# rvolden/C3POa

Measured on AMD Instinct MI355X. Metric: R2C2 reads->consensus/sec, higher is better.
Workload: dtype int32

## Files before the change

c3poa_amd/csrc/c3_api.hip:

```cpp
#include "c3_dev.h"
#include "c3_args.h"
#include <algorithm>
#include <cstddef>
#include <cstdio>
#include <cstring>
#include <string>
#include <vector>

extern "C" void c3k_launch_conk(const ConkArgs*, int, int, int, hipStream_t);
extern "C" void c3k_launch_adapter(const AdapterArgs*, int, hipStream_t);
extern "C" void c3k_launch_pairwise(const uint8_t*, int, const uint8_t*, int, const uint8_t*, int, uint8_t*, uint8_t*, int*, hipStream_t);
extern "C" void c3k_launch_match_index(const char*, const int*, int, int, const char*, const long long*, int*, hipStream_t);
extern "C" void c3k_launch_demux(const uint8_t*, int, const uint8_t*, int, int, int, int32_t*, uint8_t*, hipStream_t);
extern "C" void c3k_launch_peaks(const PeaksArgs*, int, hipStream_t);
extern "C" int c3k_peaks_blocks_per_cu(void);
extern "C" void c3k_launch_poa(const PoaArgs*, int, int, int, hipStream_t);
extern "C" void c3k_launch_prep(const PrepArgs*, int, hipStream_t);
extern "C" void c3k_launch_window(const WinArgs*, int, hipStream_t);
extern "C" void c3k_launch_stitch(const StitchArgs*, int, hipStream_t);
extern "C" void c3k_launch_zero(const ZeroArgs*, int, hipStream_t);
extern "C" void c3k_launch_zero_long(const ZeroArgs*, int, hipStream_t);
extern "C" void c3k_launch_zero_finish(const ZeroArgs*, int, hipStream_t);
extern "C" void c3k_launch_qv(const QvArgs*, int, hipStream_t);
extern "C" int c3k_qv_lds_max(void);
// ... 506 lines not shown
  if ((rc = run_zero(h))) return rc;
  const int n = h->n;
  h->work.clear();
  for (int i = 0; i < n; ++i) if (h->sum[i].status == C3_ST_OK && h->sum[i].n_sub >= 1) h->work.push_back(i);
  if (n < (1 << 24)) {
    const size_t m = h->work.size();
    std::vector<uint64_t> keys(m), tmp(m);
    for (size_t k = 0; k < m; ++k) {
      const int i = h->work[k];
      const uint64_t cost = (uint64_t)h->sum[i].sum_sub * (uint64_t)h->sum[i].n_sub;
      keys[k] = ((((uint64_t)1 << 40) - 1 - cost) << 24) | (uint64_t)i;
    }
    uint64_t* src = keys.data(); uint64_t* dst = tmp.data();
    for (int pass = 0; pass < 4; ++pass) {
      const int sh = 24 + 10 * pass;
      size_t cnt[1025] = {0};
      for (size_t k = 0; k < m; ++k) ++cnt[((src[k] >> sh) & 1023) + 1];
      for (int b = 0; b < 1024; ++b) cnt[b + 1] += cnt[b];
      for (size_t k = 0; k < m; ++k) dst[cnt[(src[k] >> sh) & 1023]++] = src[k];
      std::swap(src, dst);
    }
    for (size_t k = 0; k < m; ++k) h->work[k] = (int)(src[k] & 0xffffff);
  } else {
    std::stable_sort(h->work.begin(), h->work.end(), [&](int x, int y) {
      long cx = (long)h->sum[x].sum_sub * h->sum[x].n_sub, cy = (long)h->sum[y].sum_sub * h->sum[y].n_sub; return cx > cy; });
  }
  HIPCHK(h->d_work.ensure(sizeof(int) * std::max<size_t>(h->work.size(), 1)));
  if (!h->work.empty()) HIPCHK(hipMemcpyAsync(h->d_work.p, h->work.data(), sizeof(int) * h->work.size(), hipMemcpyHostToDevice, h->stream));
  return 0;
}

static int launch_poa(c3_handle* h, const int* d_work, int nw, int Ncap, int K, int Pcap, long long cells, int* d_overflow, int* d_overflow16, int waves_per_cu, int wide_ring) {
  const size_t N = (size_t)Ncap;
  const int NI = 19;
  cells = (cells + 15) & ~15LL;
  cells = (cells + 63) & ~63LL;
  const bool w32 = d_overflow16 == nullptr || getenv("C3_DEBUG_POA32");
  const long long far = w32 ? cells : cells >> 2;
  const size_t per_slot = N * (NI * 4 + 8 + 5 + 32 + 4 * C3_JUMP_LEVELS) + N * K * 12 + (size_t)cells * 2 + (size_t)far * 16 + (size_t)Pcap * 4;
  const int slots = auto_slots(h, h->cfg.slots_poa, per_slot, nw, waves_per_cu);
  HIPCHK(h->s_poa_i.ensure(sizeof(int) * N * NI * slots)); HIPCHK(h->s_poa_nk.ensure(sizeof(int) * N * K * 3 * slots));
  HIPCHK(h->s_poa_cells.ensure(((size_t)cells * 2 + (size_t)far * 16) * slots + 256)); HIPCHK(h->s_poa_b.ensure(N * 5 * slots)); HIPCHK(h->s_poa_sc.ensure(sizeof(long long) * N * slots));
  HIPCHK(h->s_poa_desc.ensure(sizeof(uint4) * 2 * N * slots));
  HIPCHK(h->s_poa_jump.ensure(sizeof(int) * C3_JUMP_LEVELS * N * slots));
  HIPCHK(h->s_poa_path.ensure(sizeof(int) * (size_t)Pcap * slots));
  PoaArgs a; memset(&a, 0, sizeof(a));
  a.b = dev_batch(h); a.info = h->d_info.as<C3Info>(); a.p = dev_params(h->cfg);
  a.counter = h->d_counter.as<int>(); a.work = d_work; a.n_work = nw;
  a.ibase = h->s_poa_i.as<int>(); a.ebase = h->s_poa_nk.as<int>(); a.cellsb = h->s_poa_cells.as<char>();
  a.bbase = h->s_poa_b.as<uint8_t>(); a.score = h->s_poa_sc.as<long long>();
  a.Ncap = Ncap; a.K = K; a.Pcap = Pcap; a.cells_cap = (int)cells; a.desc = h->s_poa_desc.as<uint4>(); a.jump = h->s_poa_jump.as<int>();
  a.pbase = h->s_poa_path.as<int>(); a.overflow = d_overflow; a.overflow16 = d_overflow16;
  if (const char* e = getenv("C3_DEBUG_POA_RBSPAN")) a.rb_span = std::max(3300, atoi(e));
  a.draft = h->d_draft.as<uint8_t>(); a.tpos = h->d_tpos.as<int32_t>();
  a.msa_dbg = nullptr; a.msa_off = nullptr; a.msa_len = nullptr;
  if (h->debug_msa) { a.msa_dbg = h->d_msa.as<uint8_t>(); a.msa_off = h->d_msa_off.as<int64_t>(); a.msa_len = h->d_msa_len.as<int>(); }
  a.phases = (unsigned long long*)(h->d_counter.as<char>() + 64);
  DBG("poa: nw=%d Ncap=%d K=%d cells=%lld slots=%d (%.1f MB per slot)%s\n", nw, Ncap, K, cells, slots, per_slot / 1048576.0, d_overflow ? "" : (d_overflow16 ? " [full-size pass]" : " [32-bit pass]"));
  c3k_launch_poa(&a, slots, w32 ? 1 : 0, wide_ring, h->stream);
  HIPCHK(hipGetLastError());
  return 0;
}

static int run_poa(c3_handle* h) {
  const int nw = (int)h->work.size();
  HIPCHK(h->d_draft.ensure((size_t)h->total + 64)); HIPCHK(h->d_tpos.ensure(sizeof(int32_t) * (size_t)h->total + 64));
  HIPCHK(h->d_cons.ensure((size_t)h->total + 64));
  HIPCHK(hipMemsetAsync(h->d_tpos.p, 0xff, sizeof(int32_t) * (size_t)h->total, h->stream));
  if (nw == 0) return 0;
  int max_sum = 0, max_ns = 0, max_q = 0;
  for (int i : h->work) { max_sum = std::max(max_sum, h->sum[i].sum_sub); max_ns = std::max(max_ns, h->sum[i].n_sub); max_q = std::max(max_q, h->sum[i].max_sub); }
  const int Ncap_full = max_sum + 8, K = max_ns + 1, Pcap = max_sum + 8;
  const int w = h->cfg.poa_band_b + (int)(h->cfg.poa_band_f * max_q);
  long long cells_full = (long long)(2 * max_q + 2) * (2 * w + 1 + max_q / 5);
  if (max_ns < 2) cells_full = 64;
  if (cells_full > 0x7fffff00LL) cells_full = 0x7fffff00LL;
  const double nodes_typ = (double)max_q * (1.0 + 0.15 * std::max(0, max_ns - 1));
  int Ncap = (int)std::min<double>(Ncap_full, 1.3 * nodes_typ + 256);
  long long cells = std::min<long long>(cells_full, (long long)(1.5 * nodes_typ * (2 * w + 12)) + 4096);
  if (const char* e_ = getenv("C3_DEBUG_POA_SMALL")) { Ncap = std::min(Ncap_full, std::max(64, atoi(e_))); cells = std::min<long long>(cells_full, 16LL * Ncap); }
  if (h->debug_msa) {
    std::vector<int64_t> mo(h->n + 1, 0);
    for (int i = 0; i < h->n; ++i) mo[i + 1] = mo[i] + (int64_t)h->sum[i].n_sub * (h->sum[i].sum_sub + 2);
    HIPCHK(h->d_msa.ensure((size_t)mo[h->n] + 64)); HIPCHK(h->d_msa_off.ensure(sizeof(int64_t) * (h->n + 1))); HIPCHK(h->d_msa_len.ensure(sizeof(int) * h->n));
    HIPCHK(hipMemcpyAsync(h->d_msa_off.p, mo.data(), sizeof(int64_t) * (h->n + 1), hipMemcpyHostToDevice, h->stream));
    HIPCHK(hipMemsetAsync(h->d_msa_len.p, 0, sizeof(int) * h->n, h->stream));
    HIPCHK(hipStreamSynchronize(h->stream));
  }
  HIPCHK(h->d_overflow.ensure(sizeof(int) * 2 * (size_t)nw));
  HIPCHK(hipMemsetAsync(h->d_counter.p, 0, 4, h->stream));
  HIPCHK(hipMemsetAsync(h->d_counter.as<char>() + 16, 0, 240, h->stream));
  int wide_ring = (max_q > 1792 || 2 * w + 1 + 24 > 128) ? 1 : 0;
  if (const char* e_ = getenv("C3_DEBUG_POA_WIDE")) wide_ring = atoi(e_) ? 1 : 0;
  int* ovA = h->d_overflow.as<int>(); int* ovB = h->d_overflow.as<int>() + nw;
  int rc = launch_poa(h, h->d_work.as<int>(), nw, Ncap, K, Pcap, cells, ovA, ovB, 24, wide_ring);
  if (rc) return rc;
  h->n_poa_redo = 0; h->n_poa_redo16 = 0;
  {
    int cnt[8];
    HIPCHK(hipMemcpyAsync(cnt, h->d_counter.p, 32, hipMemcpyDeviceToHost, h->stream));
    HIPCHK(hipStreamSynchronize(h->stream));
    if (cnt[4] > 0) {
      h->n_poa_redo = cnt[4];
      HIPCHK(hipMemsetAsync(h->d_counter.p, 0, 4, h->stream));
      if ((rc = launch_poa(h, ovA, cnt[4], Ncap_full, K, Pcap, cells_full, nullptr, ovB, 24, wide_ring))) return rc;
      HIPCHK(hipMemcpyAsync(cnt, h->d_counter.p, 32, hipMemcpyDeviceToHost, h->stream));
// ... 751 lines not shown
```

c3poa_amd/csrc/c3_args.h:

```cpp
#pragma once
#include "c3_dev.h"

struct ConkArgs {
  C3Batch b; const uint8_t* sp_codes; const int* sp_len; int32_t* track; C3Info* info; int* counter;
  int match, mismatch, penalty;
  int n_spl; int32_t* scan;
};
struct PeaksArgs {
  C3Batch b; const int32_t* track; C3Info* info; double* bufA; double* bufB; int32_t* cand; uint8_t* cstate;
  int32_t* raw_peaks; int32_t* n_raw; const int* sp_len; double coef[64]; int64_t maxL; int window, iters, min_dist;
  int* queue;
};
struct PoaArgs {
  C3Batch b; C3Info* info; C3Params p; int* counter; const int* work; int n_work;
  int* ibase; int* ebase; char* cellsb; uint8_t* bbase; long long* score;
  int Ncap, K, Pcap, cells_cap;
  uint8_t* draft; int32_t* tpos; uint8_t* msa_dbg; const int64_t* msa_off; int* msa_len;
  unsigned long long* phases; uint4* desc; int* jump;
  int* pbase;
  int* overflow;
  int* overflow16;
  int rb_span;
};
struct WLayer { int qbeg, len, begin, end; };
struct WinRec { int rid, w, n_layers, blen, tgs, out_len, polished, pad_; };
struct PrepArgs {
  C3Batch b; C3Info* info; C3Params p; int* counter; const int* work; int n_work;
  const uint8_t* draft; int32_t* tpos; int32_t* eH; uint8_t* eD; int64_t ecap; int* lw_first; int* lw_last; int NLcap, NWcap;
  WinRec* wrec; WLayer* wlay; int* win_base; int* n_windows; int wcap;
};
struct WinArgs {
  C3Batch b; C3Params p; int* counter; int n_win; const WinRec* wrec_in; WinRec* wrec; const WLayer* wlay; int NLcap;
  const uint8_t* draft;
  uint8_t* base; int* ibase; int* ebase; long long* score;
  int32_t* H; uint16_t* D; uint4* rdesc; int Ncap, K; long long hcap; uint8_t* wout; int wout_cap;
  int Lcap;
  unsigned long long* phases;
  int band_mode;
  const int* wlist; const int* n_win_dev; int* ovf_list;
};
#define W_CNT_OVF 48
#define W_CNT_Q2 49
struct StitchArgs {
  C3Batch b; C3Info* info; const int* work; int n_work; const WinRec* wrec; const int* win_base; const uint8_t* wout; int wout_cap; char* cons;
  const uint8_t* zflag;
};
struct AdapterArgs {
  C3Batch b; C3Params p; int* counter;
  const uint8_t* ad_codes; const int* ad_len; int n_ad;
  uint8_t* D; long long dcap;
  int32_t* out;
};

struct ZeroArgs {
  C3Batch b; C3Info* info; C3Params p; int* counter; const int* work; int n_work;
  uint8_t* D; long long dcap;
  int4* zinfo; uint8_t* zflag;
  const uint8_t* draft; char* cons;
  uint8_t* S; long long scap; int zk;
};

struct ZlLayout { long long ck, dir, car, total; };
__host__ __device__ inline ZlLayout c3_zl_layout(long long n0, long long n1, long long K) {
  ZlLayout l;
  l.ck = 0;
  l.dir = (n1 + K - 1) / K * (n0 + 1) * 8;
  l.car = (l.dir + (n1 < K ? n1 : K) * (n0 + 1) + 15) & ~15LL;
  l.total = (l.car + n1 * 12 + 255) & ~255LL;
  return l;
}
struct QvArgs {
  int n_reads; const C3Info* info; const uint32_t* pk; const int64_t* woff; const uint8_t* qual; const int64_t* off;
  const char* cons; char* qv;
  int sa_np, sa_n; const int64_t* sa_woff; const int64_t* sa_off; const int32_t* sa_mode;
  uint32_t* dirs; long long dir_words;
// ... 5 lines not shown
```

c3poa_amd/csrc/k_poa.hip:

```cpp
#include "c3_dev.h"
#include "c3_args.h"
#include <type_traits>

#define WSYNC() __syncthreads()
#define EI(v, k) ((size_t)(k) * (size_t)c.Ncap + (size_t)(v))
#define C3_POA_NI 19
#define SRC 0
#define SNK 1


struct Ctx {
  int* I; int* E; char* C; uint8_t* B8; long long* score_; uint4* desc_; int* jump_; int* path_;
  int K, n, Ncap, cells_cap;
  int far_shift;
  int osel;
  int rb_span;
  const uint32_t* pk;
#ifdef C3_DEBUG_PUNT
  unsigned long long* dbg;
#endif
#define CTX_I(name, k) __device__ __forceinline__ int* name() const { return I + (size_t)(k) * Ncap; }
  CTX_I(n_in, 0) CTX_I(n_out, 1) CTX_I(grp, 2) CTX_I(index, 5) CTX_I(gfirst, 6) CTX_I(glast, 7)
  CTX_I(rem, 8) CTX_I(mpl, 9) CTX_I(mpr, 10) CTX_I(rowm, 11)  CTX_I(anchor, 14) CTX_I(col, 15)
  CTX_I(col2t, 16) CTX_I(nxt, 17) CTX_I(foff, 18)
#undef CTX_I
  __device__ __forceinline__ int* order() const { return I + (size_t)(3 + osel) * Ncap; }
  __device__ __forceinline__ int* order2() const { return I + (size_t)(4 - osel) * Ncap; }
  __device__ __forceinline__ int* in_from() const { return E; }
  __device__ __forceinline__ int* out_to() const { return E + (size_t)Ncap * K; }
  __device__ __forceinline__ int* out_w() const { return E + 2 * (size_t)Ncap * K; }
  __device__ __forceinline__ int far_cap() const { return cells_cap >> far_shift; }
  __device__ __forceinline__ int32_t* H() const { return (int32_t*)(C + 2 * (size_t)cells_cap); }
  __device__ __forceinline__ int32_t* E1() const { return (int32_t*)(C + 2 * (size_t)cells_cap + 4 * (size_t)far_cap()); }
  __device__ __forceinline__ int32_t* E2() const { return (int32_t*)(C + 2 * (size_t)cells_cap + 8 * (size_t)far_cap()); }
  __device__ __forceinline__ uint32_t* D() const { return (uint32_t*)(C + 2 * (size_t)cells_cap + 12 * (size_t)far_cap()); }
  __device__ __forceinline__ uint8_t* D8() const { return (uint8_t*)C; }
  __device__ __forceinline__ uint8_t* P8() const { return (uint8_t*)(C + (size_t)cells_cap); }
  __device__ __forceinline__ uint8_t* base() const { return B8; }
  __device__ __forceinline__ uint8_t* rows2() const { return B8 + (size_t)Ncap; }
  __device__ __forceinline__ long long* score() const { return score_; }
  __device__ __forceinline__ uint4* descA() const { return desc_; }
  __device__ __forceinline__ uint4* descB() const { return desc_ + (size_t)Ncap; }
  __device__ __forceinline__ int* jump() const { return jump_; }
  __device__ __forceinline__ int* path() const { return path_; }
};

__device__ __forceinline__ void g_add_edge(Ctx& c, int u, int v, int w) {
  const int K = c.K;
  for (int k = 0; k < c.n_out()[u]; ++k)
    if (c.out_to()[EI(u, k)] == v) { c.out_w()[EI(u, k)] += w; return; }
  int no = c.n_out()[u], ni = c.n_in()[v];
  c.out_to()[EI(u, no)] = v; c.out_w()[EI(u, no)] = w; c.n_out()[u] = no + 1;
  c.in_from()[EI(v, ni)] = u; c.n_in()[v] = ni + 1;
}

#ifndef GU
#define GU 2
#endif
__device__ void g_blocks(Ctx& c, int lane) {
  int gprev = -1;
  for (int i0 = 0; i0 < c.n; i0 += 64 * GU) {
    int v[GU], r[GU];
#pragma unroll
    for (int u = 0; u < GU; ++u) { const int i = i0 + 64 * u + lane; v[u] = i < c.n ? c.order()[i] : -1; }
#pragma unroll
    for (int u = 0; u < GU; ++u) r[u] = v[u] >= 0 ? c.grp()[v[u]] : -2;
#pragma unroll
    for (int u = 0; u < GU; ++u) {
      const int i = i0 + 64 * u + lane;
// ... 153 lines not shown
  const int w = wave_first(P.band_b + (int)(P.band_f * (double)Q));
  const int le1_8 = e1_8 * lane, le2_8 = e2_8 * lane;
#define le1 (le1_8 << 6)
#define le2 (le2_8 << 6)
  const int lo1_8 = le1_8 + o1_8, lo2_8 = le2_8 + o2_8;
  const bool qlds = WIDE || Q <= PQW_N * 16;
  poa_sweep_desc(c, lane, Q, qlds, PR);
  int qwb = 0;
  auto stage_query = [&](int from) {
    for (int i = lane; i < PQW && from + 16 * i < Q; i += 64) {
      const long long b0 = (long long)qb + from + 16 * i;
      const unsigned w0 = c.pk[b0 >> 4], w1 = c.pk[(b0 >> 4) + 1];
      Lqpk[i] = __builtin_amdgcn_alignbit(w1, w0, (unsigned)(b0 & 15) * 2);
    }
  };
  if (qlds) stage_query(0);
  if (!W32) { unsigned* r32 = (unsigned*)&L.ring[0]; for (int i = lane; i < 3 * RING_CELLS / 2; i += 64) r32[i] = NEG16 | (NEG16 << 16); }
  WSYNC();
  PH_MARK(0)
  int u_beg = 0, u_end = -1, u_left = 0, u_right = 0, u_ncell = 0;
  int u_b8 = 0;
  int u_nfar = 0;
  int pH = NEG16, pE1 = NEG16, pE2 = NEG16;
  bool pv_ok = false;
  int gacc = 0xffff;
  int punt = 0;
  const int lane4 = lane * 4;
  unsigned short* const LH = &L.ring[0]; unsigned short* const LE1 = &L.ring[RING_CELLS]; unsigned short* const LE2 = &L.ring[2 * RING_CELLS];
#ifdef C3_EXP_SBAND
#define UNI(x)
#else
#define UNI(x) asm volatile("" : "+v"(x))
#endif
#ifdef C3_PHASE_PROF
  unsigned long long row_t0 = __builtin_readcyclecounter();
#endif
  int slot = PR - 1;
  for (int ib = 0; ib < n; ib += 64) {
  uint4 dA = c.descA()[min(ib + lane, n - 1)], dB = c.descB()[min(ib + lane, n - 1)];
  asm volatile("" : "+v"(dA.x), "+v"(dA.y), "+v"(dA.z), "+v"(dA.w), "+v"(dB.x), "+v"(dB.y), "+v"(dB.z), "+v"(dB.w));
  const int cnt = min(64, n - ib);
  for (int li = 0; li < cnt; ++li) {
    const int idx = ib + li;
    slot = slot == PR - 1 ? 0 : slot + 1;
    const int fl = __builtin_amdgcn_readlane(dA.z, li);
    if ((fl >> 19) & 1) { pv_ok = false; continue; }
    const int qr = __builtin_amdgcn_readlane(dA.w, li);
    const int vb = fl & 0xff;
    const bool far = W32 || ((fl >> 16) & 1);
    if (WIDE && qr + w + 72 > qwb + PQW * 16 && qwb + PQW * 16 < Q) {
      qwb = max(0, qr - w - 320) & ~15;
      WSYNC(); stage_query(qwb); WSYNC();
    }
    if (!W32 && ((fl >> 18) & 1) && pv_ok) {
      UNI(u_beg); UNI(u_end); UNI(u_left); UNI(u_right); UNI(u_ncell);
      const bool nonempty = u_end >= u_beg;
      const int mplv = nonempty ? u_left + 1 : INT32_MAX / 2, mprv = nonempty ? u_right + 1 : 0;
      const int beg = max(max(0, min(mplv, qr) - w), u_beg);
      int end = min(min(Q, max(mprv, qr) + w), u_end + 1);
      end = max(end, beg - 1);
      const int wd = end - beg + 1, sh = beg - u_beg;
      if (__builtin_amdgcn_ballot_w64(((int)((unsigned)(wd - 1) < 64u) & (int)(wd + sh <= 64) & ((int)(sh >= 1) | (int)(u_end - u_beg < 63)) & (int)(u_ncell + 64 <= c.cells_cap) & (int)(!far || u_nfar + 64 <= c.far_cap()) & (int)(!WIDE || (max(beg - 1, 0) >= qwb && end <= qwb + PQW * 16))) != 0) != 0) {
        const int ro = u_ncell;
        const int j = beg + lane;
        const bool act = lane < wd;
        const int jq = max(j - 1, 0) - (WIDE ? qwb : 0);
        const unsigned qw_ = Lqpk[min(jq >> 4, PQW - 1)];
        const int a_p = lane4 + sh * 4, a_d = a_p - 4;
        const int hd = __builtin_amdgcn_ds_bpermute(a_d, pH), hp = __builtin_amdgcn_ds_bpermute(a_p, pH);
        const int e1p = __builtin_amdgcn_ds_bpermute(a_p, pE1), e2p = __builtin_amdgcn_ds_bpermute(a_p, pE2);
        const int qc = (int)((qw_ >> ((jq & 15) * 2)) & 3);
        const int M = hd + ((vb == qc) ? mt8 + 2 : mm8 + 2);
        const int E1t = maxu16(hp - (oe1_8 - 1), e1p - e1_8);
        const int E2t = maxu16(hp - (oe2_8 - 2), e2p - e2_8);
        const int E1c = E1t & ~7, E2c = E2t & ~7;
        const int k2 = maxu16(maxu16(M, E1c + 1), E2c);
        const int ht = k2 & ~7;
        const int htm = act ? ht : NEG2_16;
        int s1 = htm + le1_8, s2 = htm + le2_8, s3 = htm;
        wave_scan_max3(s1, s2, s3);
        const int px1 = wave_shr1(s1, NEG2_16), px2 = wave_shr1(s2, NEG2_16);
        const int htl = wave_shr1(htm, NEG16);
        const int f1 = px1 - lo1_8, f2 = px2 - lo2_8;
        const int k3 = maxu16(maxu16(ht + 2, f1 + 1), f2);
        const int h = k3 & ~7;
        unsigned d = ((unsigned)E1t & 1u) | ((unsigned)E2t & 2u) | (((unsigned)k2 & 3u) << 2) | (((unsigned)k3 & 3u) << 4);
        d |= (((unsigned)(htl - oe1_8 - f1)) >> 25) & 64u;
        d |= (((unsigned)(htl - oe2_8 - f2)) >> 24) & 128u;
        const int rb = __builtin_amdgcn_readlane(s3, 63);
        const unsigned long long mxm = __ballot(htm == rb);
        const int left = beg + __builtin_ctzll(mxm), right = beg + (63 - __builtin_clzll(mxm));
        pH = maxu16(act ? h : NEG16, FLOOR16); pE1 = act ? E1c : NEG16; pE2 = act ? E2c : NEG16;
        int nb8 = u_b8;
        if ((unsigned)(rb - RB_LO16) > (unsigned)c.rb_span) {
          const int m1 = rb - BIAS16, fl1 = FLOOR16 + max(m1, 0);
          nb8 += m1; punt |= (int)(rb < GLO16);
          pH = act ? maxu16(h, fl1) - m1 : NEG16; pE1 = act ? maxu16(E1c, fl1) - m1 : NEG16; pE2 = act ? maxu16(E2c, fl1) - m1 : NEG16;
        }
        gacc = minu16(gacc, pH - (ZHI16 + 1));
#ifdef C3_DEBUG_PUNT
        if (pH > ZHI16 && pH < GLO16) { atomicAdd(c.dbg + 8, 1ull); atomicMax(c.dbg + 9, ((unsigned long long)(65535 - pH) << 40) | ((unsigned long long)idx << 16) | ((unsigned long long)lane << 8) | (unsigned long long)(wd & 255)); atomicMax(c.dbg + 10, ((unsigned long long)(65535 - pH) << 40) | ((unsigned long long)(unsigned short)rb << 16) | (unsigned)(sh & 255) << 8 | (unsigned)(u_end - u_beg + 1)); }
#endif
        c.D8()[(unsigned)(ro + lane)] = (uint8_t)d;
        { const int cb = slot * PWT + PADL + lane;
          LH[cb] = (unsigned short)pH; LE1[cb] = (unsigned short)pE1; LE2[cb] = (unsigned short)pE2;
#pragma unroll
          for (int f = 1; f < NCHMAX; ++f) { LH[cb + 64 * f] = NEG16; LE1[cb + 64 * f] = NEG16; LE2[cb + 64 * f] = NEG16; }
        }
        if (lane == 0) {
          L.meta[slot] = make_int4(beg, end, left, right); L.base8[slot] = nb8;
          int off = 3 * idx; UNI(off);
          int* rm = c.rowm() + off; rm[0] = beg; rm[1] = end; rm[2] = ro;
        }
        if (far) {
          const int fo = wave_first(u_nfar);
          if (act) { c.H()[fo + lane] = cv_16to9(pH, nb8); c.E1()[fo + lane] = cv_16to9(pE1, nb8); c.E2()[fo + lane] = cv_16to9(pE2, nb8); }
          if (lane == 0) { c.mpl()[idx] = left; c.mpr()[idx] = right; c.foff()[idx] = fo; }
          u_nfar = fo + wave_first(wd);
        }
        u_beg = beg; u_end = end; u_left = left; u_right = right; u_ncell = ro + wd; u_b8 = nb8;
#ifdef C3_PHASE_PROF
        { unsigned long long t_ = __builtin_readcyclecounter(); ph_acc_[8] += t_ - row_t0; row_t0 = t_; }
#endif
        continue;
      }
    }
    const int v = __builtin_amdgcn_readlane(dA.x, li);
    const int nin = (fl >> 8) & 0xff;
    const bool ovf = (fl >> 17) & 1;
    const int p0 = __builtin_amdgcn_readlane(dB.x, li), p1 = __builtin_amdgcn_readlane(dB.y, li);
    const int p2 = __builtin_amdgcn_readlane(dB.z, li), p3 = __builtin_amdgcn_readlane(dB.w, li);
    const int psl = __builtin_amdgcn_readlane(dA.y, li);
    const int ps0 = psl & 15, ps1 = (psl >> 4) & 15, ps2 = (psl >> 8) & 15, ps3 = (psl >> 12) & 15;
#define PRED_IDX(k) ((k) == 0 ? p0 : (k) == 1 ? p1 : (k) == 2 ? p2 : (k) == 3 ? p3 : c.index()[c.in_from()[EI(v, (k))]])
#define PRED_SLOT(k) ((k) == 0 ? ps0 : (k) == 1 ? ps1 : (k) == 2 ? ps2 : ps3)
    int ncell = wave_first(u_ncell);
    if (!W32 && C3_NEAR && !ovf && qlds && v != SRC && idx - p0 < PR && (nin < 2 || idx - p1 < PR) && (nin < 3 || idx - p2 < PR) && (nin < 4 || idx - p3 < PR)) {
      auto near_body = [&](auto NPc, auto NCHc) -> bool {
      constexpr int NP = decltype(NPc)::value, NCH = decltype(NCHc)::value;
      UNI(u_ncell);
      const int BIGB = 1 << 28;
      int4 m_[NP]; int b8_[NP], sl_[NP];
#pragma unroll
      for (int k = 0; k < NP; ++k) { sl_[k] = k < nin ? PRED_SLOT(k) : 0; m_[k] = L.meta[sl_[k]]; b8_[k] = L.base8[sl_[k]]; }
      int pb_[NP], dk_[NP];
      int mplv = INT32_MAX / 2, mprv = 0, minb = INT32_MAX, maxe = INT32_MIN, wmax = 0, dabs = 0;
#pragma unroll
      for (int k = 0; k < NP; ++k) {
        const bool has = k < nin;
        const int b = has ? m_[k].x : BIGB, e = has ? m_[k].y : -BIGB;
        pb_[k] = b;
        dk_[k] = has ? b8_[k] - b8_[0] : 0;
        dabs = max(dabs, max(dk_[k], -dk_[k]));
        minb = min(minb, b); maxe = max(maxe, e + 1); wmax = max(wmax, e - b);
        const bool ne = e >= b;
        mplv = ne ? min(mplv, m_[k].z + 1) : mplv; mprv = ne ? max(mprv, m_[k].w + 1) : mprv;
      }
      const int beg = max(max(0, min(mplv, qr) - w), minb);
      int end = min(min(Q, max(mprv, qr) + w), maxe);
      end = max(end, beg - 1);
      const int wd = end - beg + 1;
      if (__builtin_amdgcn_ballot_w64(((int)((unsigned)(wd - 1) < (unsigned)(64 * NCH)) & (int)(wmax < PW) & (int)(dabs < 2048) & (int)(u_ncell + 64 * NCH <= c.cells_cap) & (int)(!far || u_nfar + 64 * NCH <= c.far_cap()) & (int)(!WIDE || (max(beg - 1, 0) >= qwb && end <= qwb + PQW * 16))) != 0) == 0) return false;
      const int ro = u_ncell;
      const int W8 = wave_first(b8_[0]);
      int cM[NP], c1o[NP], c1x[NP], c2o[NP], c2x[NP], sb_[NP];
#pragma unroll
      for (int k = 0; k < NP; ++k) {
        cM[k] = dk_[k] + (3 - k);
        c1o[k] = dk_[k] - oe1_8 + (7 - 2 * k); c1x[k] = dk_[k] - e1_8 + (6 - 2 * k);
        c2o[k] = dk_[k] - oe2_8 + (7 - 2 * k); c2x[k] = dk_[k] - e2_8 + (6 - 2 * k);
        sb_[k] = sl_[k] * PWT + PADL - pb_[k];
      }
      int carry1 = 0, carry2 = 0, prev_ht = NEG16;
      int best = 0, left = 0, right = 0;
      int cH[NCH], cE1[NCH], cE2[NCH];
#pragma unroll
      for (int ch = 0; ch < NCH; ++ch) {
        const int c0 = 64 * ch;
        const int j = beg + c0 + lane;
// ... 30 lines not shown
        const int htl = wave_shr1(htm, prev_ht);
        const int f1 = px1 - o1_8 - cl1, f2 = px2 - o2_8 - cl2;
        if (NCH > 1) { carry1 = max(carry1, wave_bcast(s1, 63)); carry2 = max(carry2, wave_bcast(s2, 63)); prev_ht = wave_bcast(htm, 63); }
        const int k3 = maxu16(maxu16(ht + 2, f1 + 1), f2);
        const int h = k3 & ~7;
        d |= (((unsigned)k3 & 3u) << 4);
        d |= (((unsigned)(htl - oe1_8 - f1)) >> 25) & 64u;
        d |= (((unsigned)(htl - oe2_8 - f2)) >> 24) & 128u;
        c.D8()[(unsigned)(ro + c0 + lane)] = (uint8_t)d; c.P8()[(unsigned)(ro + c0 + lane)] = (uint8_t)pby;
        cH[ch] = h; cE1[ch] = E1c; cE2[ch] = E2c;
        const int cmx = __builtin_amdgcn_readlane(s3, 63);
        const unsigned long long mxm = __ballot(htm == cmx);
        if (NCH == 1 || cmx > best) { best = cmx; left = beg + c0 + __builtin_ctzll(mxm); right = beg + c0 + (63 - __builtin_clzll(mxm)); }
        else if (cmx == best && mxm) right = beg + c0 + (63 - __builtin_clzll(mxm));
      }
      int nb8 = W8;
      if ((unsigned)(best - RB_LO16) > (unsigned)c.rb_span) {
        const int m1 = best - BIAS16, fl1 = FLOOR16 + max(m1, 0);
        nb8 += m1; punt |= (int)(best < GLO16);
#pragma unroll
        for (int ch = 0; ch < NCH; ++ch) { cH[ch] = maxu16(cH[ch], fl1) - m1; cE1[ch] = maxu16(cE1[ch], fl1) - m1; cE2[ch] = maxu16(cE2[ch], fl1) - m1; }
      }
#pragma unroll
      for (int ch = 0; ch < NCH; ++ch) {
        const bool act = 64 * ch + lane < wd;
        const int vH = maxu16(act ? cH[ch] : NEG16, FLOOR16), vE1 = act ? cE1[ch] : NEG16, vE2 = act ? cE2[ch] : NEG16;
        gacc = minu16(gacc, vH - (ZHI16 + 1));
#ifdef C3_DEBUG_PUNT
        if (vH > ZHI16 && vH < GLO16) { atomicAdd(c.dbg + 11, 1ull); atomicMax(c.dbg + 12, ((unsigned long long)(65535 - vH) << 40) | ((unsigned long long)idx << 16) | ((unsigned long long)lane << 8) | (unsigned long long)(wd & 255)); }
#endif
        const int cb = slot * PWT + PADL + 64 * ch + lane;
        LH[cb] = (unsigned short)vH; LE1[cb] = (unsigned short)vE1; LE2[cb] = (unsigned short)vE2;
        if (ch == NCH - 1) {
#pragma unroll
          for (int f = 1; f <= NCHMAX - NCH; ++f) { LH[cb + 64 * f] = NEG16; LE1[cb + 64 * f] = NEG16; LE2[cb + 64 * f] = NEG16; }
        }
        if (ch == 0) { pH = vH; pE1 = vE1; pE2 = vE2; }
        if (far) { if (act) { c.H()[u_nfar + 64 * ch + lane] = cv_16to9(vH, nb8); c.E1()[u_nfar + 64 * ch + lane] = cv_16to9(vE1, nb8); c.E2()[u_nfar + 64 * ch + lane] = cv_16to9(vE2, nb8); } }
      }
      pv_ok = NCH == 1;
      if (lane == 0) {
        L.meta[slot] = make_int4(beg, end, left, right); L.base8[slot] = nb8;
        int off = 3 * idx; UNI(off);
        int* rm = c.rowm() + off; rm[0] = beg; rm[1] = end | (1 << 28); rm[2] = ro;
        if (far) { c.mpl()[idx] = left; c.mpr()[idx] = right; c.foff()[idx] = u_nfar; }
      }
      if (far) u_nfar = wave_first(u_nfar) + wave_first(wd);
#ifdef C3_EXP_SBAND
      u_beg = wave_first(beg); u_end = wave_first(end); u_left = wave_first(left); u_right = wave_first(right); u_ncell = wave_first(ro + wd); u_b8 = nb8;
#else
      u_beg = beg; u_end = end; u_left = left; u_right = right; u_ncell = ro + wd; u_b8 = nb8;
#endif
#ifdef C3_PHASE_PROF
      { unsigned long long t_ = __builtin_readcyclecounter(); ph_acc_[10] += t_ - row_t0; row_t0 = t_; }
#endif
      return true;
      };
      typedef std::integral_constant<int, 1> I1; typedef std::integral_constant<int, 2> I2; typedef std::integral_constant<int, 3> I3; typedef std::integral_constant<int, 4> I4;
      typedef std::integral_constant<int, WIDE ? 2 : 1> CA; typedef std::integral_constant<int, WIDE ? 3 : 2> CB; typedef std::integral_constant<int, 4> CC;
      bool handled = nin == 1 ? near_body(I1{}, CA{}) : nin == 2 ? near_body(I2{}, CA{}) : nin == 3 ? near_body(I3{}, CA{}) : near_body(I4{}, CA{});
      if (!handled) handled = nin == 1 ? near_body(I1{}, CB{}) : nin == 2 ? near_body(I2{}, CB{}) : nin == 3 ? near_body(I3{}, CB{}) : near_body(I4{}, CB{});
      if (WIDE && C3_WIDE_PW >= 256) { if (!handled && nin <= 2) handled = nin == 1 ? near_body(I1{}, CC{}) : near_body(I2{}, CC{}); }
      if (handled) continue;
    }
    int beg, end;
    int pb_[4] = {0, 0, 0, 0}, pe_[4] = {-1, -1, -1, -1};
    int rb8_[4] = {0, 0, 0, 0};
    bool ring_[4] = {false, false, false, false};
    if (v == SRC) { beg = 0; end = min(Q, max(qr, 0) + w); }
    else {
      int mplv = INT32_MAX / 2, mprv = 0, minb = INT32_MAX, maxe = INT32_MIN;
      int4 m_[4]; int b8m_[4];
#pragma unroll
      for (int k = 0; k < 4; ++k) { m_[k] = L.meta[PRED_SLOT(k)]; b8m_[k] = L.base8[PRED_SLOT(k)]; }
      asm volatile("" : "+v"(m_[0].x), "+v"(m_[1].x), "+v"(m_[2].x), "+v"(m_[3].x));
#pragma unroll
      for (int k = 0; k < 4; ++k) {
        if (k < nin) {
          const int pi = k == 0 ? p0 : k == 1 ? p1 : k == 2 ? p2 : p3;
          int b = m_[k].x, e = m_[k].y, l = m_[k].z, r = m_[k].w;
          if (W32 || idx - pi >= PR) { b = c.rowm()[3 * pi]; e = c.rowm()[3 * pi + 1] & 0x0fffffff; l = c.mpl()[pi]; r = c.mpr()[pi]; }
          b = wave_first(b); e = wave_first(e); l = wave_first(l); r = wave_first(r);
          pb_[k] = b; pe_[k] = e; ring_[k] = !W32 && idx - pi < PR && e - b + 1 <= PW; rb8_[k] = wave_first(b8m_[k]);
          minb = min(minb, b); maxe = max(maxe, e + 1);
          if (e >= b) { mplv = min(mplv, l + 1); mprv = max(mprv, r + 1); }
        }
      }
      for (int k = 4; k < nin; ++k) {
        const int pi = PRED_IDX(k);
        const int sl = pi % PR;
        int4 m = L.meta[sl];
        asm volatile("" : "+v"(m.x), "+v"(m.y), "+v"(m.z), "+v"(m.w));
        int b = m.x, e = m.y, l = m.z, r = m.w;
        if (W32 || idx - pi >= PR) { b = c.rowm()[3 * pi]; e = c.rowm()[3 * pi + 1] & 0x0fffffff; l = c.mpl()[pi]; r = c.mpr()[pi]; }
        minb = min(minb, b); maxe = max(maxe, e + 1);
        if (e >= b) { mplv = min(mplv, l + 1); mprv = max(mprv, r + 1); }
      }
      beg = max(0, min(mplv, qr) - w);
      end = min(Q, max(mprv, qr) + w);
      beg = max(beg, minb); end = min(end, maxe);
    }
    beg = wave_first(beg); end = wave_first(end);
    if (end < beg) end = beg - 1;
    const int wd = end - beg + 1;
#ifdef C3_DEBUG_PUNT
    if (ncell + wd > c.cells_cap && lane == 0) atomicAdd(c.dbg + 12, 1ull);
#endif
// ... 325 lines not shown
    if (row[si] != 4) { out[n++] = qual[qi]; ++qi; ++si; }
    else if (qi == 0) { out[n++] = qual[qi]; ++si; }
    else { out[n++] = (uint8_t)(((int)qual[qi - 1] + (int)qual[qi]) / 2); ++si; }
  }
  if (n != msa_len) { int gap = 0; while (gap < msa_len && row[msa_len - 1 - gap] == 4) { out[n] = out[n - 1]; ++n; ++gap; } }
}

__device__ int pairwise_merge(const uint8_t* rowA, const uint8_t* rowB, int ncol, const uint8_t* qa, const uint8_t* qb_,
                              uint8_t* draft, int* col2t) {
  int o = 0, i = 0;
  while (i != ncol) {
    const int A = rowA[i], B = rowB[i];
    if (A == B) { if (A != 4) { if (col2t) col2t[i] = o; draft[o++] = (uint8_t)A; } }
    if (A != B && A != 4 && B != 4) { if (col2t) col2t[i] = o; draft[o++] = (uint8_t)((qa[i] > qb_[i]) ? A : B); }
    if (A == 4 || B == 4) {
      int gl = 1; const uint8_t* gs = (A == 4) ? rowA : rowB;
      for (;;) { if (i + gl >= ncol) { gl = 1; break; } if (gs[i + gl] == 4) ++gl; else break; }
      long sa = 0, sb = 0;
      for (int k = i; k < i + gl && k < ncol; ++k) { sa += qa[k]; sb += qb_[k]; }
      const uint8_t* srcr = (sa > sb) ? rowA : rowB;
      for (int k = i; k < i + gl && k < ncol; ++k) if (srcr[k] != 4) { if (col2t) col2t[k] = o; draft[o++] = srcr[k]; }
      i += gl; continue;
    }
    ++i;
  }
  return o;
}

__global__ void k_pairwise(const uint8_t* rows, int ncol, const uint8_t* qualA, int lenA, const uint8_t* qualB, int lenB,
                           uint8_t* scratch, uint8_t* out, int* out_len) {
  if (threadIdx.x != 0 || blockIdx.x != 0) return;
  normalize_len(rows, ncol, qualA, lenA, scratch);
  normalize_len(rows + ncol, ncol, qualB, lenB, scratch + ncol);
  out_len[0] = pairwise_merge(rows, rows + ncol, ncol, scratch, scratch + ncol, out, nullptr);
}
extern "C" void c3k_launch_pairwise(const uint8_t* rows, int ncol, const uint8_t* qa, int la, const uint8_t* qb, int lb,
                                    uint8_t* scratch, uint8_t* out, int* out_len, hipStream_t s) {
  hipLaunchKernelGGL(k_pairwise, dim3(1), dim3(64), 0, s, rows, ncol, qa, la, qb, lb, scratch, out, out_len);
}

#ifndef C3_POA_WAVES
#define C3_POA_WAVES 6
#endif
template <bool W32, bool DEF, bool WIDE>
__global__ __launch_bounds__(64, C3_POA_WAVES) void k_poa(PoaArgs a) {
  const int lane = wave_lane();
  const int slot = blockIdx.x;
  Ctx c;
  const size_t N = (size_t)a.Ncap;
  c.I = a.ibase + (size_t)slot * C3_POA_NI * N; c.path_ = a.pbase + (size_t)slot * a.Pcap; c.E = a.ebase + (size_t)slot * 3 * N * a.K;
  c.far_shift = W32 ? 0 : 2;
  c.C = a.cellsb + (size_t)slot * (2 * (size_t)a.cells_cap + 16 * (size_t)(a.cells_cap >> c.far_shift)); c.B8 = a.bbase + (size_t)slot * 5 * N;
  c.score_ = a.score + (size_t)slot * N; c.desc_ = a.desc + (size_t)slot * 2 * N; c.jump_ = a.jump + (size_t)slot * C3_JUMP_LEVELS * N;
  c.K = a.K; c.Ncap = a.Ncap; c.cells_cap = a.cells_cap; c.osel = 0; c.rb_span = a.rb_span > 0 ? a.rb_span : RB_HI16 - RB_LO16;
#ifdef C3_DEBUG_PUNT
  c.dbg = a.phases;
#endif
  PH_DECL

  for (;;) {
    int wi = 0;
    if (lane == 0) wi = atomicAdd(a.counter, 1);
    wi = wave_first(wi);
    if (wi >= a.n_work) break;
    const int rid = a.work[wi];
    C3Info* info = &a.info[rid];
    const int ns = info->n_sub;
    const int64_t off = a.b.off[rid];
    c.pk = a.b.pk + a.b.woff[rid];
    uint8_t* draft = a.draft + off;
    int32_t* tpos = a.tpos + off;
    const uint8_t* qual = a.b.qual + off;
    long long cells = 0;
    int C = 0, fail = 0; bool punted = false;
    if (ns == 1) {
      const int qb = info->sub_beg[0]; C = info->sub_end[0] - qb;
      for (int k = lane; k < C; k += 64) { draft[k] = (uint8_t)c3_code_at(c.pk, qb + k); tpos[qb + k] = k; }
    } else {
      c.osel = 0;
      if (lane == 0) {
        c.base()[SRC] = 0; c.base()[SNK] = 0; c.n_in()[SRC] = c.n_out()[SRC] = c.n_in()[SNK] = c.n_out()[SNK] = 0;
        c.grp()[SRC] = SRC; c.grp()[SNK] = SNK; c.order()[0] = SRC; c.order()[1] = SNK; c.index()[SRC] = 0; c.index()[SNK] = 1;
      }
      c.n = 2;
      WSYNC();
      g_blocks(c, lane);
      int poff = 0;
      for (int s = 0; s < ns && !fail; ++s) {
        const int qb = wave_first(info->sub_beg[s]), Q = wave_first(info->sub_end[s]) - qb;
        if (s > 0) { const int rc = poa_align<W32, DEF, WIDE>(c, a.p, qb, Q, lane, &cells PHP); if (rc < 0) { fail = (rc == -4 || rc == -5) ? 2 : 1; punted = rc == -5; break; } }
        if (poa_fuse(c, s == 0, qb, Q, c.path() + poff, lane PHP) < 0) { fail = 2; break; }
        poff += Q;
      }
      PH_MARK(9)
      if (!fail) {
        int ncol_acc = 0;
        for (int i0 = 0; i0 < c.n; i0 += 64) {
          const int i = i0 + lane;
          int v = -1, start = 0;
          if (i < c.n) {
            v = c.order()[i];
            if (v != SRC && v != SNK) start = (i == 0) || (c.grp()[v] != c.grp()[c.order()[i - 1]]) || c.order()[i - 1] == SRC;
          }
          const int ps = wave_scan_add(start);
          if (i < c.n) c.col()[v] = (v == SRC || v == SNK) ? -1 : ncol_acc + ps - 1;
          ncol_acc += wave_bcast(ps, 63);
        }
// ... 159 lines not shown
```

Before: 404,700.

## Add two-columns-per-lane fast path for single-predecessor POA rows up to 128 wide

Adds a new fast path in the 16-bit POA DP kernel for rows with one predecessor whose band is 65–128 cells wide. Each lane computes two adjacent cells and a single wave-wide max scan resolves the horizontal gap recurrences, so these rows no longer fall through to the general multi-chunk row body. An environment variable can disable the path. The path adds register pressure and code size to the kernel, and it only fires for non-wide, non-32-bit passes.

```diff
diff --git a/c3poa_amd/csrc/c3_api.hip b/c3poa_amd/csrc/c3_api.hip
--- a/c3poa_amd/csrc/c3_api.hip
+++ b/c3poa_amd/csrc/c3_api.hip
@@ -582,6 +582,7 @@
   a.Ncap = Ncap; a.K = K; a.Pcap = Pcap; a.cells_cap = (int)cells; a.desc = h->s_poa_desc.as<uint4>(); a.jump = h->s_poa_jump.as<int>();
   a.pbase = h->s_poa_path.as<int>(); a.overflow = d_overflow; a.overflow16 = d_overflow16;
   if (const char* e = getenv("C3_DEBUG_POA_RBSPAN")) a.rb_span = std::max(3300, atoi(e));
+  a.no2col = getenv("C3_DEBUG_POA_NO2COL") != nullptr;
   a.draft = h->d_draft.as<uint8_t>(); a.tpos = h->d_tpos.as<int32_t>();
   a.msa_dbg = nullptr; a.msa_off = nullptr; a.msa_len = nullptr;
   if (h->debug_msa) { a.msa_dbg = h->d_msa.as<uint8_t>(); a.msa_off = h->d_msa_off.as<int64_t>(); a.msa_len = h->d_msa_len.as<int>(); }
diff --git a/c3poa_amd/csrc/c3_args.h b/c3poa_amd/csrc/c3_args.h
--- a/c3poa_amd/csrc/c3_args.h
+++ b/c3poa_amd/csrc/c3_args.h
@@ -21,6 +21,7 @@
   int* overflow;
   int* overflow16;
   int rb_span;
+  int no2col;
 };
 struct WLayer { int qbeg, len, begin, end; };
 struct WinRec { int rid, w, n_layers, blen, tgs, out_len, polished, pad_; };
diff --git a/c3poa_amd/csrc/k_poa.hip b/c3poa_amd/csrc/k_poa.hip
--- a/c3poa_amd/csrc/k_poa.hip
+++ b/c3poa_amd/csrc/k_poa.hip
@@ -15,6 +15,7 @@
   int far_shift;
   int osel;
   int rb_span;
+  int two_col;
   const uint32_t* pk;
 #ifdef C3_DEBUG_PUNT
   unsigned long long* dbg;
@@ -274,14 +275,16 @@
       qwb = max(0, qr - w - 320) & ~15;
       WSYNC(); stage_query(qwb); WSYNC();
     }
+#define C3_BAND_OF_ROW_ABOVE \
+      UNI(u_beg); UNI(u_end); UNI(u_left); UNI(u_right); UNI(u_ncell); \
+      const bool nonempty = u_end >= u_beg; \
+      const int mplv = nonempty ? u_left + 1 : INT32_MAX / 2, mprv = nonempty ? u_right + 1 : 0; \
+      const int beg = max(max(0, min(mplv, qr) - w), u_beg); \
+      int end = min(min(Q, max(mprv, qr) + w), u_end + 1); \
+      end = max(end, beg - 1); \
+      const int wd = end - beg + 1, sh = beg - u_beg;
     if (!W32 && ((fl >> 18) & 1) && pv_ok) {
-      UNI(u_beg); UNI(u_end); UNI(u_left); UNI(u_right); UNI(u_ncell);
-      const bool nonempty = u_end >= u_beg;
-      const int mplv = nonempty ? u_left + 1 : INT32_MAX / 2, mprv = nonempty ? u_right + 1 : 0;
-      const int beg = max(max(0, min(mplv, qr) - w), u_beg);
-      int end = min(min(Q, max(mprv, qr) + w), u_end + 1);
-      end = max(end, beg - 1);
-      const int wd = end - beg + 1, sh = beg - u_beg;
+      C3_BAND_OF_ROW_ABOVE
       if (__builtin_amdgcn_ballot_w64(((int)((unsigned)(wd - 1) < 64u) & (int)(wd + sh <= 64) & ((int)(sh >= 1) | (int)(u_end - u_beg < 63)) & (int)(u_ncell + 64 <= c.cells_cap) & (int)(!far || u_nfar + 64 <= c.far_cap()) & (int)(!WIDE || (max(beg - 1, 0) >= qwb && end <= qwb + PQW * 16))) != 0) != 0) {
         const int ro = u_ncell;
         const int j = beg + lane;
@@ -342,11 +345,84 @@
         }
         u_beg = beg; u_end = end; u_left = left; u_right = right; u_ncell = ro + wd; u_b8 = nb8;
 #ifdef C3_PHASE_PROF
-        { unsigned long long t_ = __builtin_readcyclecounter(); ph_acc_[8] += t_ - row_t0; row_t0 = t_; }
+        { unsigned long long t_ = __builtin_readcyclecounter(); ph_acc_[8] += t_ - row_t0; row_t0 = t_; ph_acc_[12] += 1; }
 #endif
         continue;
       }
     }
+    if (!WIDE && !W32 && ((fl >> 18) & 1) && c.two_col) {
+      C3_BAND_OF_ROW_ABOVE
+      if (__builtin_amdgcn_ballot_w64(((int)((unsigned)(wd - 65) < 64u) & (int)((unsigned)(u_end - u_beg) < (unsigned)PW) & (int)(u_ncell + 128 <= c.cells_cap) & (int)(!far || u_nfar + 128 <= c.far_cap())) != 0) != 0) {
+        const int ro = u_ncell;
+        int c0l = 2 * lane; UNI(c0l);
+        const bool act0 = c0l < wd, act1 = c0l + 1 < wd;
+        const int j0 = beg + c0l;
+        const int jq0 = max(j0 - 1, 0), jq1 = j0;
+        const unsigned qw0 = Lqpk[min(jq0 >> 4, PQW - 1)], qw1 = Lqpk[min(jq1 >> 4, PQW - 1)];
+        const int rx = (slot == 0 ? PR - 1 : slot - 1) * PWT + PADL + sh + c0l;
+        const int hd0 = LH[rx - 1], hp0 = LH[rx], hp1 = LH[rx + 1];
+        const int e1p0 = LE1[rx], e1p1 = LE1[rx + 1], e2p0 = LE2[rx], e2p1 = LE2[rx + 1];
+        const int qc0 = (int)((qw0 >> ((jq0 & 15) * 2)) & 3), qc1 = (int)((qw1 >> ((jq1 & 15) * 2)) & 3);
+        const int M0 = hd0 + ((vb == qc0) ? mt8 + 2 : mm8 + 2), M1 = hp0 + ((vb == qc1) ? mt8 + 2 : mm8 + 2);
+        const int E1t0 = maxu16(hp0 - (oe1_8 - 1), e1p0 - e1_8), E1t1 = maxu16(hp1 - (oe1_8 - 1), e1p1 - e1_8);
+        const int E2t0 = maxu16(hp0 - (oe2_8 - 2), e2p0 - e2_8), E2t1 = maxu16(hp1 - (oe2_8 - 2), e2p1 - e2_8);
+        const int E1c0 = E1t0 & ~7, E2c0 = E2t0 & ~7, E1c1 = E1t1 & ~7, E2c1 = E2t1 & ~7;
+        const int k20 = maxu16(maxu16(M0, E1c0 + 1), E2c0), k21 = maxu16(maxu16(M1, E1c1 + 1), E2c1);
+        const int ht0 = k20 & ~7, ht1 = k21 & ~7;
+        const int htm0 = act0 ? ht0 : NEG2_16, htm1 = act1 ? ht1 : NEG2_16;
+        const int l1 = e1_8 * c0l, l2 = e2_8 * c0l;
+        const int t10 = htm0 + l1, t20 = htm0 + l2;
+        int s1 = max(t10, htm1 + l1 + e1_8), s2 = max(t20, htm1 + l2 + e2_8), s3 = max(htm0, htm1);
+        wave_scan_max3(s1, s2, s3);
+        const int px1 = wave_shr1(s1, NEG2_16), px2 = wave_shr1(s2, NEG2_16);
+        const int f10 = px1 - o1_8 - l1, f20 = px2 - o2_8 - l2;
+        const int f11 = max(px1, t10) - (o1_8 + e1_8) - l1, f21 = max(px2, t20) - (o2_8 + e2_8) - l2;
+        const int htl0 = wave_shr1(htm1, NEG16);
+        const int k30 = maxu16(maxu16(ht0 + 2, f10 + 1), f20), k31 = maxu16(maxu16(ht1 + 2, f11 + 1), f21);
+        const int h0 = k30 & ~7, h1 = k31 & ~7;
+        unsigned d0 = ((unsigned)E1t0 & 1u) | ((unsigned)E2t0 & 2u) | (((unsigned)k20 & 3u) << 2) | (((unsigned)k30 & 3u) << 4);
+        unsigned d1 = ((unsigned)E1t1 & 1u) | ((unsigned)E2t1 & 2u) | (((unsigned)k21 & 3u) << 2) | (((unsigned)k31 & 3u) << 4);
+        d0 |= (((unsigned)(htl0 - oe1_8 - f10)) >> 25) & 64u; d0 |= (((unsigned)(htl0 - oe2_8 - f20)) >> 24) & 128u;
+        d1 |= (((unsigned)(htm0 - oe1_8 - f11)) >> 25) & 64u; d1 |= (((unsigned)(htm0 - oe2_8 - f21)) >> 24) & 128u;
+        const int rb = __builtin_amdgcn_readlane(s3, 63);
+        const unsigned long long mx0 = __ballot(htm0 == rb), mx1 = __ballot(htm1 == rb);
+        const int left = beg + min(mx0 ? 2 * (int)__builtin_ctzll(mx0) : 256, mx1 ? 2 * (int)__builtin_ctzll(mx1) + 1 : 256);
+        const int right = beg + max(mx0 ? 2 * (63 - (int)__builtin_clzll(mx0)) : -1, mx1 ? 2 * (63 - (int)__builtin_clzll(mx1)) + 1 : -1);
+        int vH0 = maxu16(act0 ? h0 : NEG16, FLOOR16), vE10 = act0 ? E1c0 : NEG16, vE20 = act0 ? E2c0 : NEG16;
+        int vH1 = maxu16(act1 ? h1 : NEG16, FLOOR16), vE11 = act1 ? E1c1 : NEG16, vE21 = act1 ? E2c1 : NEG16;
+        int nb8 = u_b8;
+        if ((unsigned)(rb - RB_LO16) > (unsigned)c.rb_span) {
+          const int m1 = rb - BIAS16, fl1 = FLOOR16 + max(m1, 0);
+          nb8 += m1; punt |= (int)(rb < GLO16);
+          vH0 = act0 ? maxu16(h0, fl1) - m1 : NEG16; vE10 = act0 ? maxu16(E1c0, fl1) - m1 : NEG16; vE20 = act0 ? maxu16(E2c0, fl1) - m1 : NEG16;
+          vH1 = act1 ? maxu16(h1, fl1) - m1 : NEG16; vE11 = act1 ? maxu16(E1c1, fl1) - m1 : NEG16; vE21 = act1 ? maxu16(E2c1, fl1) - m1 : NEG16;
+        }
+        gacc = minu16(minu16(gacc, vH0 - (ZHI16 + 1)), vH1 - (ZHI16 + 1));
+        c.D8()[(unsigned)(ro + c0l)] = (uint8_t)d0; c.D8()[(unsigned)(ro + c0l + 1)] = (uint8_t)d1;
+        { const int cb = slot * PWT + PADL + c0l;
+          LH[cb] = (unsigned short)vH0; LE1[cb] = (unsigned short)vE10; LE2[cb] = (unsigned short)vE20;
+          LH[cb + 1] = (unsigned short)vH1; LE1[cb + 1] = (unsigned short)vE11; LE2[cb + 1] = (unsigned short)vE21; }
+        if (lane == 0) {
+          L.meta[slot] = make_int4(beg, end, left, right); L.base8[slot] = nb8;
+          int off = 3 * idx; UNI(off);
+          int* rm = c.rowm() + off; rm[0] = beg; rm[1] = end; rm[2] = ro;
+        }
+        if (far) {
+          const int fo = wave_first(u_nfar);
+          if (act0) { c.H()[fo + c0l] = cv_16to9(vH0, nb8); c.E1()[fo + c0l] = cv_16to9(vE10, nb8); c.E2()[fo + c0l] = cv_16to9(vE20, nb8); }
+          if (act1) { c.H()[fo + c0l + 1] = cv_16to9(vH1, nb8); c.E1()[fo + c0l + 1] = cv_16to9(vE11, nb8); c.E2()[fo + c0l + 1] = cv_16to9(vE21, nb8); }
+          if (lane == 0) { c.mpl()[idx] = left; c.mpr()[idx] = right; c.foff()[idx] = fo; }
+          u_nfar = fo + wave_first(wd);
+        }
+        u_beg = beg; u_end = end; u_left = left; u_right = right; u_ncell = ro + wd; u_b8 = nb8;
+        pv_ok = false;
+#ifdef C3_PHASE_PROF
+        { unsigned long long t_ = __builtin_readcyclecounter(); ph_acc_[15] += t_ - row_t0; row_t0 = t_; ph_acc_[12] += 1ull << 32; }
+#endif
+        continue;
+      }
+    }
+#undef C3_BAND_OF_ROW_ABOVE
     const int v = __builtin_amdgcn_readlane(dA.x, li);
     const int nin = (fl >> 8) & 0xff;
     const bool ovf = (fl >> 17) & 1;
@@ -483,7 +559,9 @@
       u_beg = beg; u_end = end; u_left = left; u_right = right; u_ncell = ro + wd; u_b8 = nb8;
 #endif
 #ifdef C3_PHASE_PROF
-      { unsigned long long t_ = __builtin_readcyclecounter(); ph_acc_[10] += t_ - row_t0; row_t0 = t_; }
+      { unsigned long long t_ = __builtin_readcyclecounter(); ph_acc_[10] += t_ - row_t0;
+        ph_acc_[13] += NCH == 1 ? 1ull : (1ull << 32); if (NCH > 1) ph_acc_[14] += t_ - row_t0;
+        row_t0 = t_; }
 #endif
       return true;
       };
@@ -915,7 +993,7 @@
   c.far_shift = W32 ? 0 : 2;
   c.C = a.cellsb + (size_t)slot * (2 * (size_t)a.cells_cap + 16 * (size_t)(a.cells_cap >> c.far_shift)); c.B8 = a.bbase + (size_t)slot * 5 * N;
   c.score_ = a.score + (size_t)slot * N; c.desc_ = a.desc + (size_t)slot * 2 * N; c.jump_ = a.jump + (size_t)slot * C3_JUMP_LEVELS * N;
-  c.K = a.K; c.Ncap = a.Ncap; c.cells_cap = a.cells_cap; c.osel = 0; c.rb_span = a.rb_span > 0 ? a.rb_span : RB_HI16 - RB_LO16;
+  c.K = a.K; c.Ncap = a.Ncap; c.cells_cap = a.cells_cap; c.osel = 0; c.rb_span = a.rb_span > 0 ? a.rb_span : RB_HI16 - RB_LO16; c.two_col = !a.no2col;
 #ifdef C3_DEBUG_PUNT
   c.dbg = a.phases;
 #endif
```

Measured after the change: 414,500, median of 6. 1.02x the previous value.
